# 1601339895/Image-Restoration

Measured on AMD Instinct MI355X. Metric: Mpixels/sec train (Restormer base 256x256, bs 32/GPU), higher is better.
Workload: dtype bf16; 1 GPU; Restormer base (dim 48, blocks [4,6,6,8], 26.13M params) train step: fwd + L1 + bwd + AdamW, 256x256 patches, bs 32/GPU, bf16 activations, fp32 params/grads/optimizer; per_gpu_batch=32, global_batch=32, patch=256, parallelism=dp1, hip_graph=False

## Files before the change

image_restoration_amd/_lib.py:

```python
from __future__ import annotations

import ctypes as C
import os
from typing import Optional

HERE = os.path.dirname(os.path.abspath(__file__))
LIB_PATH = os.environ.get("MI_RESTORE_LIB") or os.path.join(HERE, "libmi_restore.so")

MI_F32, MI_BF16 = 0, 1
c_i64 = C.c_int64
vp = C.c_void_p
fp = C.c_void_p


class PwDesc(C.Structure):
    _fields_ = [("x1", vp), ("x1_bs", c_i64), ("x1_gs", c_i64), ("k1", C.c_int),
                ("x2", vp), ("x2_bs", c_i64), ("x2_gs", c_i64), ("k2", C.c_int),
                ("w", fp), ("w_bs", c_i64), ("w_gs", c_i64), ("w_sm", c_i64), ("w_sk", c_i64),
                ("bias", fp), ("bias_gs", c_i64),
                ("r", vp), ("r_bs", c_i64), ("r_gs", c_i64),
                ("y", vp), ("y_bs", c_i64), ("y_gs", c_i64),
                ("m", C.c_int), ("n", c_i64), ("batch", C.c_int), ("groups", C.c_int), ("dtype", C.c_int),
                ("ln_w", fp), ("ln_b", fp), ("ln_mean", fp), ("ln_rstd", fp), ("ln_mode", C.c_int),
                ("f8", C.c_int), ("f8_sx", C.c_float), ("f8_sw", C.c_float),
# ... 189 lines not shown
    "mi_gdfn_fwd_f8_ok": (C.c_int, [C.POINTER(GdfnShape), C.c_int]),
    "mi_gdfn_fwd_f8": (C.c_int, [C.POINTER(GdfnShape), C.POINTER(GdfnParams), C.POINTER(LnHead), C.POINTER(F8Scales), vp, vp, vp,
                                 vp, vp]),
    "mi_box_down": (C.c_int, [vp, vp, C.c_int, C.c_int, C.c_int, C.c_int, C.c_int, C.c_int, vp]),
    "mi_fre_rect": (C.c_int, [fp, fp, fp, vp, C.c_int, C.c_int, C.c_int, C.c_int, C.c_int, C.c_int, vp]),
    "mi_fre_split_coef_bytes": (C.c_size_t, [C.c_int, C.c_int]),
    "mi_fre_split_workspace": (C.c_size_t, [C.c_int, C.c_int, C.c_int, C.c_int]),
    "mi_fre_split_max_hw": (C.c_int, []),
    "mi_fre_split_fwd": (C.c_int, [vp, vp, vp, vp, fp, C.c_int, C.c_int, C.c_int, C.c_int, C.c_int, vp]),
    "mi_fre_split_bwd": (C.c_int, [vp, vp, fp, vp, vp, vp, C.c_int, C.c_int, C.c_int, C.c_int, C.c_int, vp, vp]),
    "mi_chan_maxmean_fwd": (C.c_int, [vp, vp, vp, C.c_int, C.c_int, c_i64, C.c_int, vp]),
    "mi_chan_maxmean_bwd": (C.c_int, [vp, vp, vp, C.c_int, C.c_int, c_i64, C.c_int, vp]),
    "mi_plane_max_fwd": (C.c_int, [vp, fp, vp, C.c_int, c_i64, C.c_int, vp]),
    "mi_pool_pair_bwd": (C.c_int, [fp, fp, vp, vp, C.c_int, c_i64, C.c_int, vp]),
    "mi_chan_gate_fwd": (C.c_int, [fp, fp, fp, fp, fp, fp, C.c_int, C.c_int, C.c_int, vp]),
    "mi_chan_gate_bwd": (C.c_int, [fp, fp, fp, fp, fp, fp, fp, fp, fp, fp, fp, C.c_int, C.c_int, C.c_int, C.c_int, vp]),
    "mi_refine_mix_fwd": (C.c_int, [vp, vp, vp, fp, vp, C.c_int, C.c_int, c_i64, C.c_int, vp]),
    "mi_refine_mix_bwd": (C.c_int, [vp, vp, vp, fp, vp, vp, vp, vp, fp, C.c_int, C.c_int, c_i64, C.c_int, vp]),
    "mi_scale_add_fwd": (C.c_int, [vp, vp, fp, fp, vp, C.c_int, C.c_int, c_i64, C.c_int, vp]),
    "mi_scale_add_bwd": (C.c_int, [vp, vp, fp, fp, vp, vp, vp, fp, fp, C.c_int, C.c_int, c_i64, C.c_int, C.c_int, vp]),
    "mi_bwd_tail_ok": (C.c_int, [C.c_int, C.c_int, c_i64, C.c_int]),
    "mi_bwd_tail_workspace": (C.c_size_t, [C.c_int, C.c_int]),
    "mi_bwd_tail_plan": (C.c_int, [C.c_int, C.c_int, C.c_int, c_i64, C.c_int, C.POINTER(c_i64)]),
    "mi_bwd_tail": (C.c_int, [vp, C.c_int, vp, C.c_int, vp, fp, fp, fp, fp, fp, vp, fp, fp, fp, C.c_int, c_i64, C.c_int,
                              C.c_int, vp, vp]),
    "mi_mdta_bwd_ln_ok": (C.c_int, [C.POINTER(MdtaShape), C.c_int]),
    "mi_mdta_bwd_ln_workspace": (C.c_size_t, [C.POINTER(MdtaShape)]),
    "mi_mdta_bwd_ln": (C.c_int, [C.POINTER(MdtaShape), C.POINTER(MdtaParams), C.POINTER(LnTail), vp, vp, vp,
                                 C.POINTER(MdtaGrads), vp, vp, vp]),
    "mi_gdfn_bwd_ln_ok": (C.c_int, [C.POINTER(GdfnShape), C.c_int]),
    "mi_gdfn_bwd_ln_workspace": (C.c_size_t, [C.POINTER(GdfnShape)]),
    "mi_gdfn_bwd_ln": (C.c_int, [C.POINTER(GdfnShape), C.POINTER(GdfnParams), C.POINTER(LnTail), vp, vp, vp,
                                 C.POINTER(GdfnGrads), vp, vp, vp]),
    "mi_gdfn_fwd": (C.c_int, [C.POINTER(GdfnShape), C.POINTER(GdfnParams), vp, vp, vp, vp, vp, vp]),
    "mi_gdfn_bwd": (C.c_int, [C.POINTER(GdfnShape), C.POINTER(GdfnParams), vp, vp, vp, C.POINTER(GdfnGrads), vp, vp,
                              vp]),
    "mi_tksa_saved_bytes": (C.c_size_t, [C.POINTER(TksaShape)]),
    "mi_tksa_workspace": (C.c_size_t, [C.POINTER(TksaShape)]),
    "mi_tksa_fwd": (C.c_int, [C.POINTER(TksaShape), C.POINTER(MdtaParams), C.POINTER(TksaParams), vp, vp, vp, vp, vp, fp, vp]),
    "mi_tksa_bwd": (C.c_int, [C.POINTER(TksaShape), C.POINTER(MdtaParams), C.POINTER(TksaParams), vp, vp, vp, C.POINTER(MdtaGrads),
                              C.POINTER(TksaGrads), vp, vp, vp]),
    "mi_msfn_saved_bytes": (C.c_size_t, [C.POINTER(MsfnShape)]),
    "mi_msfn_workspace": (C.c_size_t, [C.POINTER(MsfnShape)]),
    "mi_msfn_fwd": (C.c_int, [C.POINTER(MsfnShape), C.POINTER(MsfnParams), vp, vp, vp, vp, vp, vp]),
    "mi_msfn_bwd": (C.c_int, [C.POINTER(MsfnShape), C.POINTER(MsfnParams), vp, vp, vp, C.POINTER(MsfnGrads), vp, vp, vp]),
    "mi_mefc_saved_bytes": (C.c_size_t, [C.POINTER(MefcShape)]),
# ... 91 lines not shown
```

image_restoration_amd/csrc/bwd_tail.hip:

```cpp
#include <limits.h>
#include <stdlib.h>

#include <type_traits>

#include <atomic>

#include "internal.h"
#include "fused_common.h"

namespace mi {
namespace {
using namespace fz;

#ifndef BT_PS_ELEMS
#define BT_PS_ELEMS 72
#endif
constexpr int BT_PS = BT_PS_ELEMS;

struct BtArgs {
  const bf16* dy;
  const bf16* x;
  const bf16* dres;
  const float* mean;
  const float* rstd;
// ... 14 lines not shown
  static constexpr int CT = C / 16;
  static constexpr int ROWS = 16 * MPW;
  static constexpr int KS = (ROWS + 31) / 32;
  static constexpr int PROWS = 32 * KS;
  static constexpr int NT = 64 * NW;
  static constexpr int XS = 68;

  static constexpr int LPP = NT / 64;
  static constexpr int CPL = C / LPP;
  static constexpr int ITEMS = C * 16 / NT;
  static constexpr int XP = C / 8;
  static constexpr int PPW = 2 * XP / NW;
  static constexpr int PATCH_E = PROWS * BT_PS;
  static constexpr int TILE_B = C * 128;
  static constexpr int OFF_XH = NW * PATCH_E * 2;
  static constexpr int OFF_DR = OFF_XH + 2 * TILE_B;
  static constexpr int OFF_ACC = OFF_DR + 2 * TILE_B;
  static constexpr int OFF_GAM = OFF_ACC + C * XS * 4;
  static constexpr int OFF_ST = OFF_GAM + C * 4;
  static constexpr int BYTES = OFF_ST + NW * 512;
  static_assert(C % 16 == 0 && (LPP == 4 || LPP == 8) && C % LPP == 0 && (C * 16) % NT == 0 && (2 * XP) % NW == 0,
                "unsupported shape");
  static_assert(C / 16 <= NW, "one wave per 16-channel output tile of the dxn product");
  static_assert(BYTES <= 160 * 1024, "LDS budget");
};


template <int C, int NW, int MPW>
__global__ __launch_bounds__(64 * NW, (BtCfg<C, NW, MPW>::BYTES <= 80 * 1024 ? 2 : 1)) void bt_kernel(BtArgs a) {
  using K = BtCfg<C, NW, MPW>;
  constexpr int CT = K::CT, KS = K::KS, PS = BT_PS, XS = K::XS, NT = K::NT, LPP = K::LPP, ITEMS = K::ITEMS;
  constexpr int XP = K::XP, PPW = K::PPW;
  extern __shared__ __attribute__((aligned(16))) unsigned char lds[];
  const int t = threadIdx.x, lane = t & 63, li = lane & 15, g = lane >> 4;
  const int wv = __builtin_amdgcn_readfirstlane(t >> 6);
  bf16* const patch = reinterpret_cast<bf16*>(lds) + wv * K::PATCH_E;
  float* const acc = reinterpret_cast<float*>(lds + K::OFF_ACC);
  float* const st = reinterpret_cast<float*>(lds + K::OFF_ST + wv * 512);
  const int m0 = wv * K::ROWS;
  const bool active = m0 < a.M;
  const u32x4 zero4 = {0u, 0u, 0u, 0u};
  const unsigned un = (unsigned)a.N;

  for (int i = lane; i < K::PATCH_E / 8; i += 64) reinterpret_cast<u32x4*>(patch)[i] = zero4;

  const bool dxn_wave = wv < CT;
  s16x8 wt[NW][KS];
#pragma unroll
  for (int o = 0; o < NW; ++o)
#pragma unroll
    for (int ks = 0; ks < KS; ++ks)
#pragma unroll
      for (int j = 0; j < 8; ++j) {
        const int ml = 32 * ks + (j < 4 ? 4 * g + j : 16 + 4 * g + j - 4), m = o * K::ROWS + ml;
        const bool ok = dxn_wave && ml < K::ROWS && m < a.M;
        const int cc = dxn_wave ? 16 * wv + li : 0;
        const float v = a.w[(ok ? m : 0) * C + cc] * a.gamma[cc];
        wt[o][ks][j] = ok ? bf_bits(v) : (short)0;
      }
  f32x4 G[MPW][CT];
  float S[MPW];
#pragma unroll
  for (int i = 0; i < MPW; ++i) {
    S[i] = 0.f;
#pragma unroll
    for (int ct = 0; ct < CT; ++ct) G[i][ct] = (f32x4){0.f, 0.f, 0.f, 0.f};
  }

  u32x4 R[MPW];
  const int rl = lane >> 2;
  auto issue_dy = [&](int tile, int h) {
    const int b = tile / a.tiles_per_image, p0 = (tile - b * a.tiles_per_image) * 64 + 32 * h;
    int ln = lane;
    asm volatile("" : "+v"(ln));
    const int rl = ln >> 2;
#pragma unroll
    for (int j = 0; j < MPW; ++j) {
      const int lim = a.M - 1 - (m0 + 16 * j);
      if (lim >= 0) {
        const bf16* base = a.dy + ((int64_t)b * a.M + m0 + 16 * j) * a.N + p0;
        const unsigned off = (unsigned)(rl < lim ? rl : lim) * un + 8u * (ln & 3);
        R[j] = *reinterpret_cast<const u32x4*>(base + off);
      }
    }
  };
  auto stage_dy = [&](int h) {
#pragma unroll
    for (int j = 0; j < MPW; ++j) {
      const int lim = a.M - 1 - (m0 + 16 * j);
      *reinterpret_cast<u32x4*>(&patch[(16 * j + rl) * PS + 32 * h + 8 * (lane & 3)]) = rl <= lim ? R[j] : zero4;
    }
// ... 30 lines not shown
    const bf16* b_lo = xh + li_ * 64 + ((k0 ^ f) << 3) + 4 * (g_ & 1);
    const bf16* b_hi = xh + li_ * 64 + (((k0 + 2) ^ f) << 3) + 4 * (g_ & 1);
#pragma unroll
    for (int i0 = 0; i0 < MPW; i0 += GRP) {
      s16x8 A[GRP];
#pragma unroll
      for (int i = 0; i < GRP; ++i) {
        const bf16* ar = ar0 + 16 * (i0 + i) * PS;
        A[i] = cat8(*reinterpret_cast<const s16x4*>(ar), *reinterpret_cast<const s16x4*>(ar + 16));
        float sm = 0.f;
#pragma unroll
        for (int j = 0; j < 8; ++j) sm += bf_s(A[i][j]);
        S[i0 + i] += sm;
      }
#pragma unroll
      for (int ct = 0; ct < CT; ++ct) {
        const s16x8 Bx = cat8(*reinterpret_cast<const s16x4*>(b_lo + ct * 16 * 64), *reinterpret_cast<const s16x4*>(b_hi + ct * 16 * 64));
#pragma unroll
        for (int i = 0; i < GRP; ++i) G[i0 + i][ct] = mfma32(A[i], Bx, G[i0 + i][ct]);
      }
    }
  };
  auto dxn_tile = [&]() {
    int ln = lane;
    asm volatile("" : "+v"(ln));
    const int li_ = ln & 15, g_ = ln >> 4, qq_ = li_ >> 2, pp_ = li_ & 3;
    f32x4 d[4];
#pragma unroll
    for (int nt = 0; nt < 4; ++nt) d[nt] = (f32x4){0.f, 0.f, 0.f, 0.f};
    const bf16* tr0 = reinterpret_cast<const bf16*>(lds) + (4 * g_ + qq_) * PS + 4 * pp_;
#pragma unroll
    for (int o = 0; o < NW; ++o) {
      if (o * K::ROWS < a.M) {
#pragma unroll
        for (int ks = 0; ks < KS; ++ks) {
          s16x4 lo[4], hi[4];
#pragma unroll
          for (int nt = 0; nt < 4; ++nt) {
            lo[nt] = tr_b16(tr0 + o * K::PATCH_E + (32 * ks) * PS + 16 * nt);
            hi[nt] = tr_b16(tr0 + o * K::PATCH_E + (32 * ks + 16) * PS + 16 * nt);
          }
          lds_wait(lo[0], hi[0], lo[1], hi[1], lo[2], hi[2], lo[3], hi[3]);
#pragma unroll
          for (int nt = 0; nt < 4; ++nt) d[nt] = mfma32(cat8(lo[nt], hi[nt]), wt[o][ks], d[nt]);
        }
      }
    }
    float* const ap0 = &acc[(16 * wv + li_) * XS + 4 * g_];
#pragma unroll
    for (int nt = 0; nt < 4; ++nt) *reinterpret_cast<f32x4*>(ap0 + 16 * nt) = d[nt];
  };

  auto ln_phase = [&](const bf16* xh, bf16* dr, f32x2 rstd_p) {
    if (a.dbg & 8) return;
    int tt = t;
    asm volatile("" : "+v"(tt));
    constexpr int L2 = 2 * LPP, CPL2 = C / L2;
    static_assert(C % L2 == 0 && (L2 == 8 || L2 == 16), "pixel-pair LayerNorm phase");
    const int px0 = 2 * (tt / L2), sub = tt % L2;
    int base[2];
    base[0] = sub * 64 + ((((px0 >> 3) ^ (sub >> 1)) & 7) << 3) + (px0 & 7);
    base[1] = sub * 64 + ((((px0 >> 3) ^ (sub >> 1) ^ (L2 == 8 ? 4 : 0)) & 7) << 3) + (px0 & 7);
    const float* const ap = &acc[sub * XS + px0];
    f32x2 gv[CPL2], xv[CPL2], s1 = {0.f, 0.f}, s2 = {0.f, 0.f};
#pragma unroll
    for (int j = 0; j < CPL2; ++j) {
      gv[j] = *reinterpret_cast<const f32x2*>(ap + L2 * j * XS);
      const unsigned xb = *reinterpret_cast<const unsigned*>(xh + base[j & 1] + L2 * j * 64);
      xv[j] = (f32x2){bf_lo(xb), bf_hi(xb)};
      s1 += gv[j];
      s2 += gv[j] * xv[j];
    }
    auto dpp = [](float v, auto ctrl) {
// ... 15 lines not shown
      s1[e] = u1 * (1.0f / C); s2[e] = u2 * (1.0f / C);
    }
#pragma unroll
    for (int j = 0; j < CPL2; ++j) {
      unsigned* const slot = reinterpret_cast<unsigned*>(dr + base[j & 1] + L2 * j * 64);
      const unsigned rb = *slot;
      const f32x2 o = rstd_p * (gv[j] - s1 - xv[j] * s2);
      *slot = pack_bf2(o[0] + bf_lo(rb), o[1] + bf_hi(rb));
    }
  };
  auto store_phase = [&](const bf16* dr, int b, int p0) {
    if (a.dbg & 16) return;
    int tt = t;
    asm volatile("" : "+v"(tt));
    const int c0 = tt >> 4, q = tt & 15;
    static_assert((NT / 32) % 8 == 0, "row step of the store loop must keep the swizzle term");
    const bf16* src = dr + c0 * 64 + ((((q >> 1) ^ (c0 >> 1)) & 7) << 3) + 4 * (q & 1);
    bf16* const ob = a.dx + (int64_t)b * C * a.N + p0 + (unsigned)c0 * un + 4u * q;
#pragma unroll
    for (int i = 0; i < ITEMS; ++i)
      MI_STREAM_ST(reinterpret_cast<u32x2*>(ob + (unsigned)(NT / 16 * i) * un), *reinterpret_cast<const u32x2*>(src + NT / 16 * i * 64));
  };

#ifdef BT_STAMP
  unsigned long long tk[12] = {0, 0, 0, 0, 0, 0, 0, 0, 0, 0, 0, 0}, t_prev = fm_clock();
#define BT_TICK(i) { const unsigned long long tn_ = fm_clock(); tk[i] += tn_ - t_prev; t_prev = tn_; }
#else
#define BT_TICK(i)
#endif
  int tile = blockIdx.x;
  if (tile < a.ntiles) {
    if (active) issue_dy(tile, 0);
    issue_x(tile, 0);
  }
  __syncthreads();
  int buf = 0, pb = 0, pp0 = 0;
  bool have_prev = false;
  f32x2 rstd_prev = {0.f, 0.f};
  for (; tile < a.ntiles; tile += gridDim.x, buf ^= 1) {
    const int b = tile / a.tiles_per_image, p0 = (tile - b * a.tiles_per_image) * 64;
    const int nxt = tile + gridDim.x;
    bf16* const xh = reinterpret_cast<bf16*>(lds + K::OFF_XH + buf * K::TILE_B);
    bf16* const dr = reinterpret_cast<bf16*>(lds + K::OFF_DR + buf * K::TILE_B);
    bf16* const xh_prev = reinterpret_cast<bf16*>(lds + K::OFF_XH + (buf ^ 1) * K::TILE_B);
    bf16* const dr_prev = reinterpret_cast<bf16*>(lds + K::OFF_DR + (buf ^ 1) * K::TILE_B);
    BT_TICK(0);
    asm volatile("s_waitcnt vmcnt(0)" ::: "memory");
    BT_TICK(1);
    if (active) stage_dy(0);
#pragma unroll
    for (int k = 0; k < PPW; ++k) {
      const int pid = wv + NW * k;
// ... 17 lines not shown
    BT_TICK(2);
    __syncthreads();
    BT_TICK(3);
    if (active) issue_dy(tile, 1);
    if (have_prev) ln_phase(xh_prev, dr_prev, rstd_prev);
    BT_TICK(4);
    __syncthreads();
    BT_TICK(5);
    if (have_prev) store_phase(dr_prev, pb, pp0);
    BT_TICK(6);
    if (active && !(a.dbg & 32)) {
      wgrad_half(0, xh);
      BT_TICK(7);
      stage_dy(1);
      wave_sync();
      BT_TICK(8);
      if (nxt < a.ntiles) issue_dy(nxt, 0);
      wgrad_half(1, xh);
    }
    BT_TICK(9);
    __syncthreads();
    BT_TICK(10);
    if (nxt < a.ntiles) issue_x(nxt, buf ^ 1);
    if (dxn_wave && !(a.dbg & 34)) dxn_tile();
    BT_TICK(11);
    __syncthreads();
    have_prev = true; pb = b; pp0 = p0; rstd_prev = rstd_p;
  }
  if (have_prev) {
    const int lb = buf ^ 1;
    bf16* const xh_l = reinterpret_cast<bf16*>(lds + K::OFF_XH + lb * K::TILE_B);
    bf16* const dr_l = reinterpret_cast<bf16*>(lds + K::OFF_DR + lb * K::TILE_B);
    ln_phase(xh_l, dr_l, rstd_prev);
    __syncthreads();
    store_phase(dr_l, pb, pp0);
  }
#ifdef BT_STAMP
  if (lane == 0) {
    float* const gp = a.gpart + (int64_t)blockIdx.x * a.M * (C + 1) + wv * 16;
#pragma unroll
    for (int i = 0; i < 12; ++i) gp[i] = (float)tk[i];
  }
  return;
#endif
  if (active) {
    float* const gp = a.gpart + (int64_t)blockIdx.x * a.M * (C + 1);
#pragma unroll
    for (int i = 0; i < MPW; ++i) {
#pragma unroll
      for (int ct = 0; ct < CT; ++ct)
#pragma unroll
        for (int r = 0; r < 4; ++r) {
          const int m = m0 + 16 * i + 4 * g + r;
          if (m < a.M) gp[(int64_t)m * (C + 1) + 16 * ct + li] = G[i][ct][r];
        }
      float sv = S[i];
      sv += __shfl_xor(sv, 16);
      sv += __shfl_xor(sv, 32);
      const int m = m0 + 16 * i + li;
      if (g == 0 && m < a.M) gp[(int64_t)m * (C + 1) + C] = sv;
    }
  }
}

// ... 33 lines not shown
  }
}

static bool bt_form(int M, int C, BtPlan* p) {
  int nw, mpw;
  const int mt = (M + 15) / 16;
  if (C == 96) { nw = 8; mpw = mt <= 24 ? 3 : 4; if (mt > 32) return false; }
  else if (C == 48) { nw = 4; mpw = mt <= 12 ? 3 : 4; if (mt > 16) return false; }
  else return false;
  p->C = C; p->NW = nw; p->MPW = mpw; p->rows = 16 * mpw; p->mpad = 16 * nw * mpw;
  p->lds = C == 96 ? (mpw == 3 ? BtCfg<96, 8, 3>::BYTES : BtCfg<96, 8, 4>::BYTES)
                   : (mpw == 3 ? BtCfg<48, 4, 3>::BYTES : BtCfg<48, 4, 4>::BYTES);
  p->grid = C == 96 ? 256 : 512;
  return true;
}
}

BtPlan bwd_tail_plan(int M, int C, int B, int64_t N, int dtype) {
  BtPlan p = {};
  if (!(dtype == MI_BF16 && B > 0 && N > 0 && N % 64 == 0 && M >= 16 && bt_form(M, C, &p))) return BtPlan{};
  p.covered = true;
  const char* e = MI_ENV(MI_BT_WIDE);
  p.pays = !(C == 96 && p.MPW == 4) || !(e && atoi(e) == 0);
  p.tiles_per_image = N / 64;
  p.tiles = (int64_t)B * p.tiles_per_image;
  p.launch = (int)(p.tiles < p.grid ? p.tiles : p.grid);
  p.passes = (int)((p.tiles + p.launch - 1) / p.launch);
  p.active = (M + p.rows - 1) / p.rows;
  const size_t mc = (size_t)M * (C + 1);
  p.ws_bytes = align_up((size_t)p.grid * mc * 4, 256) + align_up(mc * 4, 256) + align_up((size_t)REDUCE_GROUPS * mc * 4, 256);
  return p;
}

bool bwd_tail_ok(int M, int C, int64_t N, int dtype) { return bwd_tail_plan(M, C, 1, N, dtype).covered; }
bool bwd_tail_pays(int M, int C) { return bwd_tail_plan(M, C, 1, 64, MI_BF16).pays; }
size_t bwd_tail_workspace(int M, int C) { return bwd_tail_plan(M, C, 1, 64, MI_BF16).ws_bytes; }

template <int C, int NW, int MPW>
static int bt_launch(const BtArgs& a, int grid, hipStream_t st) {
  using K = BtCfg<C, NW, MPW>;
  static std::atomic<unsigned> attr_set{0};
  int dev = 0;
  MI_CHECK_HIP(hipGetDevice(&dev));
  const unsigned bit = 1u << (dev & 31);
  if (!(attr_set.load(std::memory_order_relaxed) & bit)) {
    MI_CHECK_HIP(hipFuncSetAttribute(reinterpret_cast<const void*>(&bt_kernel<C, NW, MPW>),
                                     hipFuncAttributeMaxDynamicSharedMemorySize, K::BYTES));
    attr_set.fetch_or(bit, std::memory_order_relaxed);
  }
  hipLaunchKernelGGL((bt_kernel<C, NW, MPW>), dim3(grid), dim3(64 * NW), K::BYTES, st, a);
  MI_LAUNCH_CHECK();
  return MI_OK;
}

int launch_bwd_tail(const void* dy, int M, const void* x, int C, const void* dres, const float* mean, const float* rstd,
                    const float* w, const float* gamma, const float* beta, void* dx, float* dw, float* dgamma, float* dbeta,
                    int B, int64_t N, int accumulate, void* ws, hipStream_t st) {
  const BtPlan p = bwd_tail_plan(M, C, B, N, MI_BF16);
  MI_CHECK_ARG(p.covered && p.tiles <= INT_MAX, "bwd_tail: unsupported shape M=%d C=%d B=%d N=%lld", M, C, B, (long long)N);
  MI_CHECK_ARG(dy && x && mean && rstd && w && gamma && dx && dw && dgamma && ws, "bwd_tail: null pointer");
  MI_CHECK_ARG(aligned16(dy) && aligned16(x) && aligned16(dx) && (!dres || aligned16(dres)) && aligned16(mean) && aligned16(rstd),
               "bwd_tail: operands must be 16-byte aligned");
  const size_t mc = (size_t)M * (C + 1);
  Carver cv(ws);
  float* gpart = cv.take<float>((size_t)p.grid * mc * 4);
  float* gsum = cv.take<float>(mc * 4);
  float* tmp = cv.take<float>((size_t)REDUCE_GROUPS * mc * 4);
  BtArgs a;
  a.dy = (const bf16*)dy; a.x = (const bf16*)x; a.dres = (const bf16*)dres; a.mean = mean; a.rstd = rstd; a.w = w;
  a.gamma = gamma; a.dx = (bf16*)dx; a.gpart = gpart; a.M = M; a.mpad = p.mpad; a.N = N;
  a.tiles_per_image = (int)p.tiles_per_image; a.ntiles = (int)p.tiles;
  { const char* e = MI_ENV(MI_BT_DEBUG); a.dbg = e ? atoi(e) : 0; }
  const int grid = p.launch;
  {
    const double px = (double)B * N;
    ProfScope ps(st, K_BWD_TAIL, ((double)M + 3.0 * C) * px * 2 + 8.0 * px, 4.0 * M * C * px);
    if (C == 96 && p.MPW == 4) MI_TRY((bt_launch<96, 8, 4>(a, grid, st)));
    else if (C == 96) MI_TRY((bt_launch<96, 8, 3>(a, grid, st)));
    else if (p.MPW == 4) MI_TRY((bt_launch<48, 4, 4>(a, grid, st)));
    else MI_TRY((bt_launch<48, 4, 3>(a, grid, st)));
  }
  (void)gsum;
  float* gb = accumulate ? deferred_take((size_t)M * 2 * C, st) : nullptr;
  if (!gb) gb = tmp;
  {
    ProfScope ps(st, K_BWD_TAIL_FIN, 4.0 * (grid + 2.0) * mc, (double)grid * mc);
    hipLaunchKernelGGL(bt_finish2_kernel, dim3(M), dim3(1024), 0, st, gpart, grid, w, gamma, beta, dw, gb, M, C, accumulate);
    MI_LAUNCH_CHECK();
  }
  if (dbeta) MI_TRY(launch_reduce_rows(gb, dgamma, M, 2 * C, 2 * C, accumulate, 1.0f, st, nullptr, dbeta, C));
  else MI_TRY(launch_reduce_rows(gb, dgamma, M, C, 2 * C, accumulate, 1.0f, st, nullptr, nullptr, 0));
  return MI_OK;
}

}

extern "C" int mi_bwd_tail_ok(int M, int C, int64_t N, int dtype) { return mi::bwd_tail_ok(M, C, N, dtype) ? 1 : 0; }
extern "C" size_t mi_bwd_tail_workspace(int M, int C) { return mi::bwd_tail_workspace(M, C); }
extern "C" int mi_bwd_tail_plan(int M, int C, int B, int64_t N, int dtype, int64_t* out) {
  MI_CHECK_ARG(out, "bwd_tail_plan: null pointer");
  MI_CHECK_ARG(dtype == MI_F32 || dtype == MI_BF16, "bwd_tail_plan: bad dtype %d", dtype);
  MI_CHECK_ARG(M > 0 && B > 0 && N > 0, "bwd_tail_plan: bad shape M=%d B=%d N=%lld", M, B, (long long)N);
  const mi::BtPlan p = mi::bwd_tail_plan(M, C, B, N, dtype);
  const int64_t v[12] = {p.covered, p.pays, p.NW, p.MPW, p.rows, p.mpad, p.launch, p.tiles, p.passes, p.active, (int64_t)p.lds,
                         (int64_t)p.ws_bytes};
  memcpy(out, v, sizeof(v));
  return MI_OK;
}
extern "C" int mi_bwd_tail(const void* dy, int M, const void* x, int C, const void* dres, const float* mean, const float* rstd,
                           const float* w, const float* gamma, const float* beta, void* dx, float* dw, float* dgamma,
                           float* dbeta, int B, int64_t N, int accumulate, int dtype, void* ws, void* stream) {
  MI_CHECK_ARG(dtype == MI_BF16, "bwd_tail: bf16 activations only");
  return mi::launch_bwd_tail(dy, M, x, C, dres, mean, rstd, w, gamma, beta, dx, dw, dgamma, dbeta, B, N, accumulate, ws,
                             (hipStream_t)stream);
}
```

image_restoration_amd/csrc/common.h:

```cpp
#pragma once
#include <hip/hip_runtime.h>
#include <stdint.h>
#include <stdio.h>
#include <string.h>
#include <type_traits>

#include "../../include/mi_restore.h"

namespace mi {

typedef __bf16 bf16;
typedef unsigned short u16;
typedef __attribute__((ext_vector_type(2))) float f32x2;
typedef __attribute__((ext_vector_type(4))) float f32x4;
typedef __attribute__((ext_vector_type(2))) unsigned int u32x2;
typedef __attribute__((ext_vector_type(4))) unsigned int u32x4;
typedef __attribute__((ext_vector_type(4))) short s16x4;
typedef __attribute__((ext_vector_type(8))) short s16x8;

template <bool F8> struct MfmaOp;
template <> struct MfmaOp<false> {
  using Frag = s16x8;
  static __device__ __forceinline__ void enter() {}
  static __device__ __forceinline__ Frag cvt(const s16x8 v, float) { return v; }
  static __device__ __forceinline__ f32x4 mma(Frag a, Frag b, f32x4 c) { return __builtin_amdgcn_mfma_f32_16x16x32_bf16(a, b, c, 0, 0, 0); }
};
template <> struct MfmaOp<true> {
  using Frag = long;
  typedef short s16x2_t __attribute__((ext_vector_type(2)));
  typedef __bf16 bf16x2_t __attribute__((ext_vector_type(2)));
  static __device__ __forceinline__ void enter() { __builtin_amdgcn_s_setreg((0 << 11) | (23 << 6) | 1, 1); }
  static __device__ __forceinline__ Frag cvt(const s16x8 v, float scale) {
    s16x2_t lo = {0, 0}, hi = {0, 0};
    lo = __builtin_amdgcn_cvt_scalef32_pk_fp8_bf16(lo, __builtin_bit_cast(bf16x2_t, (s16x2_t){v[0], v[1]}), scale, false);
    lo = __builtin_amdgcn_cvt_scalef32_pk_fp8_bf16(lo, __builtin_bit_cast(bf16x2_t, (s16x2_t){v[2], v[3]}), scale, true);
    hi = __builtin_amdgcn_cvt_scalef32_pk_fp8_bf16(hi, __builtin_bit_cast(bf16x2_t, (s16x2_t){v[4], v[5]}), scale, false);
    hi = __builtin_amdgcn_cvt_scalef32_pk_fp8_bf16(hi, __builtin_bit_cast(bf16x2_t, (s16x2_t){v[6], v[7]}), scale, true);
    return (long)(unsigned long)(unsigned)__builtin_bit_cast(int, lo) | ((long)__builtin_bit_cast(int, hi) << 32);
  }
  static __device__ __forceinline__ f32x4 mma(Frag a, Frag b, f32x4 c) { return __builtin_amdgcn_mfma_f32_16x16x32_fp8_fp8(a, b, c, 0, 0, 0); }
};

#define MI_ENV_LIST(X)                                                                                                       \
  X(MI_BT_WIDE) X(MI_BT_DEBUG) X(MI_DW_LDS) X(MI_FG_CFG) X(MI_FG_DEBUG) X(MI_FG_NOXCD) X(MI_GRAM_FOLD) X(MI_GRAM_WANT)      \
  X(MI_GRAM_RECT) X(MI_GRAM_LDS) X(MI_GRAM_STREAM_ALL) X(MI_LN_FORM) X(MI_CO_STREAM) X(MI_ATTN_DQK_SPLIT)    \
  X(MI_PW_DMA) X(MI_PW_TM_EVEN) X(MI_PW_WAVE) X(MI_PW_CHUNKED) X(MI_PW_XWIDE) X(MI_PW_WAVE_WIDE) X(MI_PW_DIRECT)             \
  X(MI_PW_WAVE_TPW) X(MI_PW_XCD) X(MI_PW_TPB) X(MI_PW_B16) X(MI_FM_DEBUG) X(MI_FM_CFG) X(MI_NO_FUSED_MDTA) X(MI_NO_PW_LDS) X(MI_PW_LDS)
enum EnvId {
#define MI_ENV_ENUM(n) E_##n,
  MI_ENV_LIST(MI_ENV_ENUM)
#undef MI_ENV_ENUM
  E_ENV_COUNT
};
const char* env_get(int id);
#define MI_ENV(n) ::mi::env_get(::mi::E_##n)

void set_error(const char* fmt, ...);
#define MI_CHECK_ARG(cond, ...)                \
  do {                                         \
    if (!(cond)) {                             \
      mi::set_error(__VA_ARGS__);              \
      return MI_ERR_ARG;                       \
    }                                          \
  } while (0)
#define MI_CHECK_HIP(expr)                                                          \
  do {                                                                              \
    hipError_t e_ = (expr);                                                         \
// ... 243 lines not shown
```

image_restoration_amd/csrc/internal.h:

```cpp
#pragma once
#include <initializer_list>

#include "common.h"

namespace mi {
struct PwK {
  const void* x1; int64_t x1_bs, x1_gs; int k1;
  const void* x2; int64_t x2_bs, x2_gs; int k2;
  const float* w; int64_t w_bs, w_gs, w_sm, w_sk;
  const float* bias; int64_t bias_gs;
  const void* r; int64_t r_bs, r_gs;
  void* y; int64_t y_bs, y_gs;
  int m; int64_t n; int groups; int vec_ok;
  void* y2; int64_t y2_bs, y2_gs; int y_split;
};
enum PwFamily { PW_CHUNKED = 0, PW_RESIDENT, PW_DMA, PW_XRES, PW_STREAM, PW_XWIDE, PW_LDS };
enum PwWeights { PW_W_PACK = 0, PW_W_B16, PW_W_F32 };
struct PwPlan {
  int family;
  int tm, m_tiles, k_chunks;
  bool f8, ln;
  bool vec_ok;
  int slices, per_batch, per_group, chunk_elems;
  int64_t slice_elems;
// ... 60 lines not shown
struct DwArgs {
  const void* in;
  const void* gy;
  const float* w;
  const float* bias;
  void* out;
  void* gate;
  int Cc, H, W, hidden, tiles_x;
};
bool dws_eligible(int H, int W, int ks);
int dws_partial_rows(int B, int H, int W, int64_t planes);
void dws_plan(int H, int W, int64_t planes, int* band, int* nb, int* lpr, int* uni);
int dws_fwd(const DwArgs& a, int B, bool gate, bool flip, int dtype, hipStream_t st);
int dws_bwd(const DwArgs& dya, const void* xin, float* part, int B, bool want_dx, int* rows_out, int dtype, hipStream_t st);
int dws_gate_bwd(const DwArgs& a, const void* xin, float* part, int B, bool want_dw, int* rows_out, int dtype,
                 hipStream_t st);
int dws_gate_bwd_recompute(const DwArgs& a, float* part, int B, bool want_dw, int* rows_out, int dtype, hipStream_t st);
struct BtPlan {
  bool covered, pays;
  int C, NW, MPW, rows, mpad;
  int grid, launch;
  int64_t tiles_per_image, tiles;
  int passes, active;
  size_t lds, ws_bytes;
};
BtPlan bwd_tail_plan(int M, int C, int B, int64_t N, int dtype);
bool bwd_tail_ok(int M, int C, int64_t N, int dtype);
bool bwd_tail_pays(int M, int C);
size_t bwd_tail_workspace(int M, int C);
int launch_bwd_tail(const void* dy, int M, const void* x, int C, const void* dres, const float* mean, const float* rstd,
                    const float* w, const float* gamma, const float* beta, void* dx, float* dw, float* dgamma, float* dbeta,
                    int B, int64_t N, int accumulate, void* ws, hipStream_t st);
#define MI_HIDDEN __attribute__((visibility("hidden")))
MI_HIDDEN int pw_lds_tm(int M);
MI_HIDDEN size_t pw_lds_lds_bytes(int tm);
MI_HIDDEN int pw_lds_launch(const mi_pw_desc* d, const PwPlan& pl, void* ws, hipStream_t st);
int fused_gdfn_fwd_save(const mi_gdfn_fused_shape* s, const void* pack, const void* y, void* out, float* mean, float* rstd,
                        void* h0, void* g, hipStream_t st);
enum FgEntry { FG_INFER = 0, FG_TRAIN, FG_F8 };
enum FgFamily { FG_TILE = 0, FG_FOURTH };
struct FgPlan {
  bool covered;
  int family;
  int C, th, tw, pc, nw; bool save, f8;
  int nch, ngr;
  int tiles_x, tiles_y, S;
// ... 68 lines not shown
```

image_restoration_amd/ops.py:

```python
from __future__ import annotations

import ctypes as C
import os
from typing import Optional, Sequence, Tuple

import torch

from . import _lib as L

Tensor = torch.Tensor


def _dtype_code(dtype: torch.dtype) -> int:
    if dtype == torch.float32:
        return L.MI_F32
    if dtype == torch.bfloat16:
        return L.MI_BF16
    raise TypeError(f"activations must be float32 or bfloat16, got {dtype}")


def _dt(t: Tensor) -> int:
    return _dtype_code(t.dtype)


# ... 766 lines not shown
    gg = _f32_struct(L.MefcGrads, grads[:5], "MEFC gradient", C.cast(ga, C.POINTER(L.MefcStepGrads)), int(accumulate))
    ws = _ws(lib.mi_mefc_workspace(C.byref(s)), x.device)
    L.check(lib.mi_mefc_bwd(C.byref(s), C.byref(pp), _p(x), _p(out), _p(dout), _p(dx), C.byref(gg), _p(saved), _p(ws), _stream()),
            "mefc_bwd")
    return dx


def bwd_tail_ok(M: int, Cc: int, N: int, dtype: torch.dtype) -> bool:
    return bool(L.lib().mi_bwd_tail_ok(M, Cc, N, _dtype_code(dtype)))


BWD_TAIL_PLAN_FIELDS = ("covered", "pays", "waves", "fragments", "rows_per_wave", "mpad", "workgroups", "tiles", "passes",
                        "active_waves", "lds", "workspace")


def bwd_tail_plan(M: int, Cc: int, B: int, N: int, dtype: torch.dtype) -> dict:
    out = (L.c_i64 * 12)()
    L.check(L.lib().mi_bwd_tail_plan(M, Cc, B, N, _dtype_code(dtype), out), "bwd_tail_plan")
    p = dict(zip(BWD_TAIL_PLAN_FIELDS, out))
    p["covered"], p["pays"] = bool(p["covered"]), bool(p["pays"])
    return p


def bwd_tail(dy: Tensor, x: Tensor, dres: Optional[Tensor], mean: Tensor, rstd: Tensor, w: Tensor, gamma: Tensor,
             beta: Tensor, dw: Tensor, dgamma: Tensor, dbeta: Tensor, accumulate: bool) -> Tensor:
    _gpu(dy, x, dres, mean, rstd, w, gamma, beta, dw, dgamma, dbeta)
    B, Cc, H, W = x.shape
    M = dy.shape[1]
    dx = torch.empty_like(x)
    lib = L.lib()
    ws = _ws(lib.mi_bwd_tail_workspace(M, Cc), x.device)
    L.check(lib.mi_bwd_tail(_p(dy), M, _p(x), Cc, _p(dres), _p(mean), _p(rstd), _p(w), _p(gamma), _p(beta), _p(dx), _p(dw),
                            _p(dgamma), _p(dbeta), B, H * W, int(accumulate), _dt(x), _p(ws), _stream()), "bwd_tail")
    return dx


def _gdfn_fused_shape(x: Tensor, hidden: int, with_bias: bool) -> L.GdfnFusedShape:
    B, Cc, H, W = x.shape
    return L.GdfnFusedShape(B, Cc, hidden, H, W, int(with_bias))


def gdfn_fused_ok(x: Tensor, hidden: int, ks: int = 3) -> bool:
    if x.dtype != torch.bfloat16 or ks != 3 or not x.is_cuda:
        return False
    s = _gdfn_fused_shape(x, hidden, True)
    return bool(L.lib().mi_gdfn_fused_ok(C.byref(s)))
# ... 717 lines not shown
```

include/mi_restore.h:

```cpp
#ifndef MI_RESTORE_H
#define MI_RESTORE_H

#include <stddef.h>
#include <stdint.h>

#ifdef __cplusplus
extern "C" {
#endif

#define MI_RESTORE_VERSION 100

typedef enum { MI_F32 = 0, MI_BF16 = 1 } mi_dtype;

enum {
  MI_OK = 0,
  MI_ERR_ARG = -1,
  MI_ERR_ALIGN = -2,
  MI_ERR_HIP = -3
};

int mi_version(void);
const char* mi_last_error(void);
int mi_env_reload(void);

// ... 202 lines not shown
                   void* out, void* saved, void* ws, void* stream);
typedef struct { float x1, w1, x2, w2; } mi_f8_scales;
int mi_mdta_fwd_f8_ok(const mi_mdta_shape* s, int with_ln);
int mi_mdta_fwd_f8(const mi_mdta_shape* s, const mi_mdta_params* p, const mi_ln_head* ln, const mi_f8_scales* f8, const void* x,
                   const void* residual, void* out, void* ws, void* stream);
int mi_gdfn_fwd_f8_ok(const mi_gdfn_shape* s, int with_ln);
int mi_gdfn_fwd_f8(const mi_gdfn_shape* s, const mi_gdfn_params* p, const mi_ln_head* ln, const mi_f8_scales* f8, const void* x,
                   const void* residual, void* out, void* ws, void* stream);
int mi_gdfn_fused_fwd_f8(const mi_gdfn_fused_shape* s, const void* pack, const mi_f8_scales* f8, const void* y, void* out,
                         void* stream);

int mi_mdta_fused_ok(const mi_mdta_shape* s);
int mi_mdta_fused_pays(const mi_mdta_shape* s);
size_t mi_mdta_fused_pack_bytes(const mi_mdta_shape* s);
int mi_mdta_fused_pack(const mi_mdta_shape* s, const float* ln_w, const float* ln_b, const mi_mdta_params* p, void* pack,
                       void* stream);
size_t mi_mdta_fused_workspace(const mi_mdta_shape* s);
int mi_mdta_fused_plan(const mi_mdta_shape* s, int64_t* out);
int mi_mdta_fused_fwd(const mi_mdta_shape* s, const mi_mdta_params* p, const void* pack, int ln_with_bias, const void* x,
                      const void* residual, void* out, float* mean, float* rstd, void* ws, void* stream);
int mi_bwd_tail_ok(int M, int C, int64_t N, int dtype);
size_t mi_bwd_tail_workspace(int M, int C);
int mi_bwd_tail_plan(int M, int C, int B, int64_t N, int dtype, int64_t* out);
int mi_bwd_tail(const void* dy, int M, const void* x, int C, const void* dres, const float* mean, const float* rstd,
                const float* w, const float* gamma, const float* beta, void* dx, float* dw, float* dgamma, float* dbeta,
                int B, int64_t N, int accumulate, int dtype, void* ws, void* stream);
int mi_mdta_bwd_ln_ok(const mi_mdta_shape* s, int qkv_bias);
size_t mi_mdta_bwd_ln_workspace(const mi_mdta_shape* s);
int mi_mdta_bwd_ln(const mi_mdta_shape* s, const mi_mdta_params* p, const mi_ln_tail* ln, const void* x, const void* dout,
                   void* dx, const mi_mdta_grads* gr, const void* saved, void* ws, void* stream);
int mi_gdfn_bwd_ln_ok(const mi_gdfn_shape* s, int in_bias);
size_t mi_gdfn_bwd_ln_workspace(const mi_gdfn_shape* s);
int mi_gdfn_bwd_ln(const mi_gdfn_shape* s, const mi_gdfn_params* p, const mi_ln_tail* ln, const void* x, const void* dout,
                   void* dx, const mi_gdfn_grads* gr, const void* saved, void* ws, void* stream);

int mi_box_down(const void* img, void* out, int B, int C, int Hi, int Wi, int factor, int dtype, void* stream);
int mi_fre_rect(const float* pooled, const float* w0, const float* w2, int* half, int B, int C, int R, int H, int W, int n,
                void* stream);
size_t mi_fre_split_coef_bytes(int B, int C);
size_t mi_fre_split_workspace(int B, int C, int H, int W);
int mi_fre_split_max_hw(void);
int mi_fre_split_fwd(const void* feat, const int* half, void* high, void* low, float* coef, int B, int C, int H, int W, int dtype,
                     void* stream);
int mi_fre_split_bwd(const void* feat, const int* half, const float* coef, const void* dhigh, const void* dlow, void* dfeat, int B,
                     int C, int H, int W, int dtype, void* ws, void* stream);
int mi_chan_maxmean_fwd(const void* x, void* out, int* idx, int B, int C, int64_t N, int dtype, void* stream);
// ... 120 lines not shown
```

Before: 15.82 Mpixels/s.

## Register-block the dxn product in bwd_tail across 2x4 waves for C=96

For C=96, the backward tail kernel's dxn matrix product is redistributed so every one of the 8 waves computes: waves split into 2 channel halves by 4 K-quarters. Each wave holds multiple 16-channel weight tiles in registers and reuses each transposed LDS load across them, then the partial sums are reduced into the shared accumulator over several sync rounds. This removes the idle waves of the old one-wave-per-channel-tile scheme and cuts redundant LDS reads. The cost is extra __syncthreads rounds, read-modify-write traffic on the accumulator, and higher register pressure. It is on by default for C=96 and can be turned off with an environment variable.

```diff
diff --git a/image_restoration_amd/_lib.py b/image_restoration_amd/_lib.py
--- a/image_restoration_amd/_lib.py
+++ b/image_restoration_amd/_lib.py
@@ -235,6 +235,7 @@
     "mi_bwd_tail_ok": (C.c_int, [C.c_int, C.c_int, c_i64, C.c_int]),
     "mi_bwd_tail_workspace": (C.c_size_t, [C.c_int, C.c_int]),
     "mi_bwd_tail_plan": (C.c_int, [C.c_int, C.c_int, C.c_int, c_i64, C.c_int, C.POINTER(c_i64)]),
+    "mi_bwd_tail_product": (C.c_int, [C.c_int, C.c_int, C.c_int, c_i64, C.c_int]),
     "mi_bwd_tail": (C.c_int, [vp, C.c_int, vp, C.c_int, vp, fp, fp, fp, fp, fp, vp, fp, fp, fp, C.c_int, c_i64, C.c_int,
                               C.c_int, vp, vp]),
     "mi_mdta_bwd_ln_ok": (C.c_int, [C.POINTER(MdtaShape), C.c_int]),
diff --git a/image_restoration_amd/csrc/bwd_tail.hip b/image_restoration_amd/csrc/bwd_tail.hip
--- a/image_restoration_amd/csrc/bwd_tail.hip
+++ b/image_restoration_amd/csrc/bwd_tail.hip
@@ -60,13 +60,17 @@
   static_assert(C % 16 == 0 && (LPP == 4 || LPP == 8) && C % LPP == 0 && (C * 16) % NT == 0 && (2 * XP) % NW == 0,
                 "unsupported shape");
   static_assert(C / 16 <= NW, "one wave per 16-channel output tile of the dxn product");
+  static constexpr int CTW = CT / 2;
+  static constexpr int KQ = NW / 2;
+  static constexpr int SPQ = NW * KS / KQ;
   static_assert(BYTES <= 160 * 1024, "LDS budget");
 };
 
 
-template <int C, int NW, int MPW>
+template <int C, int NW, int MPW, int RB>
 __global__ __launch_bounds__(64 * NW, (BtCfg<C, NW, MPW>::BYTES <= 80 * 1024 ? 2 : 1)) void bt_kernel(BtArgs a) {
   using K = BtCfg<C, NW, MPW>;
+  static_assert(!RB || (K::CT % 2 == 0 && NW % 2 == 0 && NW / 2 == 4 && (NW * K::KS) % 4 == 0), "register-blocked product: 2 x 4 waves");
   constexpr int CT = K::CT, KS = K::KS, PS = BT_PS, XS = K::XS, NT = K::NT, LPP = K::LPP, ITEMS = K::ITEMS;
   constexpr int XP = K::XP, PPW = K::PPW;
   extern __shared__ __attribute__((aligned(16))) unsigned char lds[];
@@ -82,20 +86,43 @@
 
   for (int i = lane; i < K::PATCH_E / 8; i += 64) reinterpret_cast<u32x4*>(patch)[i] = zero4;
 
-  const bool dxn_wave = wv < CT;
-  s16x8 wt[NW][KS];
-#pragma unroll
-  for (int o = 0; o < NW; ++o)
-#pragma unroll
-    for (int ks = 0; ks < KS; ++ks)
-#pragma unroll
-      for (int j = 0; j < 8; ++j) {
-        const int ml = 32 * ks + (j < 4 ? 4 * g + j : 16 + 4 * g + j - 4), m = o * K::ROWS + ml;
-        const bool ok = dxn_wave && ml < K::ROWS && m < a.M;
-        const int cc = dxn_wave ? 16 * wv + li : 0;
-        const float v = a.w[(ok ? m : 0) * C + cc] * a.gamma[cc];
-        wt[o][ks][j] = ok ? bf_bits(v) : (short)0;
-      }
+  const bool dxn_wave = RB || wv < CT;
+  s16x8 wt[RB ? 1 : NW][RB ? 1 : KS];
+  const int ch = wv & 1, kq = wv >> 1;
+  const int nreal = ((a.M + K::ROWS - 1) / K::ROWS) * KS, spq = (nreal + K::KQ - 1) / K::KQ;
+  s16x8 wt2[RB ? K::SPQ : 1][RB ? K::CTW : 1];
+  if constexpr (RB) {
+#pragma unroll
+    for (int s = 0; s < K::SPQ; ++s) {
+      const int f = kq * spq + s, o = f / KS, ks = f % KS;
+      const bool step = s < spq && f < nreal;
+#pragma unroll
+      for (int c3 = 0; c3 < K::CTW; ++c3) {
+        const int cc = 16 * (K::CTW * ch + c3) + li;
+        const float gm = a.gamma[cc];
+#pragma unroll
+        for (int j = 0; j < 8; ++j) {
+          const int ml = 32 * ks + (j < 4 ? 4 * g + j : 16 + 4 * g + j - 4), m = o * K::ROWS + ml;
+          const bool ok = step && ml < K::ROWS && m < a.M;
+          const float v = a.w[(ok ? m : 0) * C + cc] * gm;
+          wt2[s][c3][j] = ok ? bf_bits(v) : (short)0;
+        }
+      }
+    }
+  } else {
+#pragma unroll
+    for (int o = 0; o < NW; ++o)
+#pragma unroll
+      for (int ks = 0; ks < KS; ++ks)
+#pragma unroll
+        for (int j = 0; j < 8; ++j) {
+          const int ml = 32 * ks + (j < 4 ? 4 * g + j : 16 + 4 * g + j - 4), m = o * K::ROWS + ml;
+          const bool ok = dxn_wave && ml < K::ROWS && m < a.M;
+          const int cc = dxn_wave ? 16 * wv + li : 0;
+          const float v = a.w[(ok ? m : 0) * C + cc] * a.gamma[cc];
+          wt[o][ks][j] = ok ? bf_bits(v) : (short)0;
+        }
+  }
   f32x4 G[MPW][CT];
   float S[MPW];
 #pragma unroll
@@ -105,6 +132,14 @@
     for (int ct = 0; ct < CT; ++ct) G[i][ct] = (f32x4){0.f, 0.f, 0.f, 0.f};
   }
 
+#ifdef BT_STAMP
+  unsigned long long tk[14] = {0, 0, 0, 0, 0, 0, 0, 0, 0, 0, 0, 0, 0, 0}, t_prev = 0;
+#define BT_TICK_RESET() t_prev = fm_clock()
+#define BT_TICK(i) { const unsigned long long tn_ = fm_clock(); tk[i] += tn_ - t_prev; t_prev = tn_; }
+#else
+#define BT_TICK_RESET()
+#define BT_TICK(i)
+#endif
   u32x4 R[MPW];
   const int rl = lane >> 2;
   auto issue_dy = [&](int tile, int h) {
@@ -181,6 +216,7 @@
     }
   };
   auto dxn_tile = [&]() {
+    if constexpr (RB) return;
     int ln = lane;
     asm volatile("" : "+v"(ln));
     const int li_ = ln & 15, g_ = ln >> 4, qq_ = li_ >> 2, pp_ = li_ & 3;
@@ -201,13 +237,61 @@
           }
           lds_wait(lo[0], hi[0], lo[1], hi[1], lo[2], hi[2], lo[3], hi[3]);
 #pragma unroll
-          for (int nt = 0; nt < 4; ++nt) d[nt] = mfma32(cat8(lo[nt], hi[nt]), wt[o][ks], d[nt]);
+          for (int nt = 0; nt < 4; ++nt) d[nt] = mfma32(cat8(lo[nt], hi[nt]), wt[RB ? 0 : o][RB ? 0 : ks], d[nt]);
         }
       }
     }
     float* const ap0 = &acc[(16 * wv + li_) * XS + 4 * g_];
 #pragma unroll
     for (int nt = 0; nt < 4; ++nt) *reinterpret_cast<f32x4*>(ap0 + 16 * nt) = d[nt];
+  };
+
+  auto dxn_tile_rb = [&](bool run) {
+    if constexpr (RB) {
+      int ln = lane;
+      asm volatile("" : "+v"(ln));
+      const int li_ = ln & 15, g_ = ln >> 4, qq_ = li_ >> 2, pp_ = li_ & 3;
+      f32x4 d[4][K::CTW];
+#pragma unroll
+      for (int j = 0; j < 4; ++j)
+#pragma unroll
+        for (int c3 = 0; c3 < K::CTW; ++c3) d[j][c3] = (f32x4){0.f, 0.f, 0.f, 0.f};
+      const bf16* tr0 = reinterpret_cast<const bf16*>(lds) + (4 * g_ + qq_) * PS + 4 * pp_;
+      if (run) {
+#pragma unroll
+        for (int s = 0; s < K::SPQ; ++s) {
+          const int f = kq * spq + s;
+          if (s < spq && f < nreal) {
+            const bf16* tr = tr0 + (f / KS) * K::PATCH_E + 32 * (f % KS) * PS;
+            s16x4 lo[4], hi[4];
+#pragma unroll
+            for (int j = 0; j < 4; ++j) {
+              const int nt = (j + kq) & 3;
+              lo[j] = tr_b16(tr + 16 * nt);
+              hi[j] = tr_b16(tr + 16 * PS + 16 * nt);
+            }
+            lds_wait(lo[0], hi[0], lo[1], hi[1], lo[2], hi[2], lo[3], hi[3]);
+#pragma unroll
+            for (int j = 0; j < 4; ++j)
+#pragma unroll
+              for (int c3 = 0; c3 < K::CTW; ++c3) d[j][c3] = mfma32(cat8(lo[j], hi[j]), wt2[s][c3], d[j][c3]);
+          }
+        }
+      }
+      BT_TICK(12);
+      float* const ap0 = &acc[(16 * K::CTW * ch + li_) * XS + 4 * g_];
+#pragma unroll
+      for (int j = 0; j < 4; ++j) {
+        if (j) __syncthreads();
+        float* const ap = ap0 + 16 * ((j + kq) & 3);
+#pragma unroll
+        for (int c3 = 0; c3 < K::CTW; ++c3) {
+          f32x4* const p = reinterpret_cast<f32x4*>(ap + 16 * c3 * XS);
+          *p = j ? *p + d[j][c3] : d[j][c3];
+        }
+      }
+      BT_TICK(13);
+    }
   };
 
   auto ln_phase = [&](const bf16* xh, bf16* dr, f32x2 rstd_p) {
@@ -269,12 +353,7 @@
       MI_STREAM_ST(reinterpret_cast<u32x2*>(ob + (unsigned)(NT / 16 * i) * un), *reinterpret_cast<const u32x2*>(src + NT / 16 * i * 64));
   };
 
-#ifdef BT_STAMP
-  unsigned long long tk[12] = {0, 0, 0, 0, 0, 0, 0, 0, 0, 0, 0, 0}, t_prev = fm_clock();
-#define BT_TICK(i) { const unsigned long long tn_ = fm_clock(); tk[i] += tn_ - t_prev; t_prev = tn_; }
-#else
-#define BT_TICK(i)
-#endif
+  BT_TICK_RESET();
   int tile = blockIdx.x;
   if (tile < a.ntiles) {
     if (active) issue_dy(tile, 0);
@@ -338,7 +417,8 @@
     __syncthreads();
     BT_TICK(10);
     if (nxt < a.ntiles) issue_x(nxt, buf ^ 1);
-    if (dxn_wave && !(a.dbg & 34)) dxn_tile();
+    if constexpr (RB) dxn_tile_rb(!(a.dbg & 34));
+    else if (dxn_wave && !(a.dbg & 34)) dxn_tile();
     BT_TICK(11);
     __syncthreads();
     have_prev = true; pb = b; pp0 = p0; rstd_prev = rstd_p;
@@ -355,7 +435,7 @@
   if (lane == 0) {
     float* const gp = a.gpart + (int64_t)blockIdx.x * a.M * (C + 1) + wv * 16;
 #pragma unroll
-    for (int i = 0; i < 12; ++i) gp[i] = (float)tk[i];
+    for (int i = 0; i < 14; ++i) gp[i] = (float)tk[i];
   }
   return;
 #endif
@@ -435,6 +515,8 @@
   p.covered = true;
   const char* e = MI_ENV(MI_BT_WIDE);
   p.pays = !(C == 96 && p.MPW == 4) || !(e && atoi(e) == 0);
+  const char* rb = MI_ENV(MI_BT_REGBLOCK);
+  p.product = C == 96 && !(rb && atoi(rb) == 0) ? 2 : 1;
   p.tiles_per_image = N / 64;
   p.tiles = (int64_t)B * p.tiles_per_image;
   p.launch = (int)(p.tiles < p.grid ? p.tiles : p.grid);
@@ -449,7 +531,7 @@
 bool bwd_tail_pays(int M, int C) { return bwd_tail_plan(M, C, 1, 64, MI_BF16).pays; }
 size_t bwd_tail_workspace(int M, int C) { return bwd_tail_plan(M, C, 1, 64, MI_BF16).ws_bytes; }
 
-template <int C, int NW, int MPW>
+template <int C, int NW, int MPW, int RB>
 static int bt_launch(const BtArgs& a, int grid, hipStream_t st) {
   using K = BtCfg<C, NW, MPW>;
   static std::atomic<unsigned> attr_set{0};
@@ -457,11 +539,11 @@
   MI_CHECK_HIP(hipGetDevice(&dev));
   const unsigned bit = 1u << (dev & 31);
   if (!(attr_set.load(std::memory_order_relaxed) & bit)) {
-    MI_CHECK_HIP(hipFuncSetAttribute(reinterpret_cast<const void*>(&bt_kernel<C, NW, MPW>),
+    MI_CHECK_HIP(hipFuncSetAttribute(reinterpret_cast<const void*>(&bt_kernel<C, NW, MPW, RB>),
                                      hipFuncAttributeMaxDynamicSharedMemorySize, K::BYTES));
     attr_set.fetch_or(bit, std::memory_order_relaxed);
   }
-  hipLaunchKernelGGL((bt_kernel<C, NW, MPW>), dim3(grid), dim3(64 * NW), K::BYTES, st, a);
+  hipLaunchKernelGGL((bt_kernel<C, NW, MPW, RB>), dim3(grid), dim3(64 * NW), K::BYTES, st, a);
   MI_LAUNCH_CHECK();
   return MI_OK;
 }
@@ -488,10 +570,13 @@
   {
     const double px = (double)B * N;
     ProfScope ps(st, K_BWD_TAIL, ((double)M + 3.0 * C) * px * 2 + 8.0 * px, 4.0 * M * C * px);
-    if (C == 96 && p.MPW == 4) MI_TRY((bt_launch<96, 8, 4>(a, grid, st)));
-    else if (C == 96) MI_TRY((bt_launch<96, 8, 3>(a, grid, st)));
-    else if (p.MPW == 4) MI_TRY((bt_launch<48, 4, 4>(a, grid, st)));
-    else MI_TRY((bt_launch<48, 4, 3>(a, grid, st)));
+    if (C == 96 && p.product == 2) {
+      if (p.MPW == 4) MI_TRY((bt_launch<96, 8, 4, 1>(a, grid, st)));
+      else MI_TRY((bt_launch<96, 8, 3, 1>(a, grid, st)));
+    } else if (C == 96 && p.MPW == 4) MI_TRY((bt_launch<96, 8, 4, 0>(a, grid, st)));
+    else if (C == 96) MI_TRY((bt_launch<96, 8, 3, 0>(a, grid, st)));
+    else if (p.MPW == 4) MI_TRY((bt_launch<48, 4, 4, 0>(a, grid, st)));
+    else MI_TRY((bt_launch<48, 4, 3, 0>(a, grid, st)));
   }
   (void)gsum;
   float* gb = accumulate ? deferred_take((size_t)M * 2 * C, st) : nullptr;
@@ -520,6 +605,11 @@
   memcpy(out, v, sizeof(v));
   return MI_OK;
 }
+extern "C" int mi_bwd_tail_product(int M, int C, int B, int64_t N, int dtype) {
+  MI_CHECK_ARG(dtype == MI_F32 || dtype == MI_BF16, "bwd_tail_product: bad dtype %d", dtype);
+  MI_CHECK_ARG(M > 0 && B > 0 && N > 0, "bwd_tail_product: bad shape M=%d B=%d N=%lld", M, B, (long long)N);
+  return mi::bwd_tail_plan(M, C, B, N, dtype).product;
+}
 extern "C" int mi_bwd_tail(const void* dy, int M, const void* x, int C, const void* dres, const float* mean, const float* rstd,
                            const float* w, const float* gamma, const float* beta, void* dx, float* dw, float* dgamma,
                            float* dbeta, int B, int64_t N, int accumulate, int dtype, void* ws, void* stream) {
diff --git a/image_restoration_amd/csrc/common.h b/image_restoration_amd/csrc/common.h
--- a/image_restoration_amd/csrc/common.h
+++ b/image_restoration_amd/csrc/common.h
@@ -42,7 +42,7 @@
 };
 
 #define MI_ENV_LIST(X)                                                                                                       \
-  X(MI_BT_WIDE) X(MI_BT_DEBUG) X(MI_DW_LDS) X(MI_FG_CFG) X(MI_FG_DEBUG) X(MI_FG_NOXCD) X(MI_GRAM_FOLD) X(MI_GRAM_WANT)      \
+  X(MI_BT_WIDE) X(MI_BT_DEBUG) X(MI_BT_REGBLOCK) X(MI_DW_LDS) X(MI_FG_CFG) X(MI_FG_DEBUG) X(MI_FG_NOXCD) X(MI_GRAM_FOLD) X(MI_GRAM_WANT)      \
   X(MI_GRAM_RECT) X(MI_GRAM_LDS) X(MI_GRAM_STREAM_ALL) X(MI_LN_FORM) X(MI_CO_STREAM) X(MI_ATTN_DQK_SPLIT)    \
   X(MI_PW_DMA) X(MI_PW_TM_EVEN) X(MI_PW_WAVE) X(MI_PW_CHUNKED) X(MI_PW_XWIDE) X(MI_PW_WAVE_WIDE) X(MI_PW_DIRECT)             \
   X(MI_PW_WAVE_TPW) X(MI_PW_XCD) X(MI_PW_TPB) X(MI_PW_B16) X(MI_FM_DEBUG) X(MI_FM_CFG) X(MI_NO_FUSED_MDTA) X(MI_NO_PW_LDS) X(MI_PW_LDS)
diff --git a/image_restoration_amd/csrc/internal.h b/image_restoration_amd/csrc/internal.h
--- a/image_restoration_amd/csrc/internal.h
+++ b/image_restoration_amd/csrc/internal.h
@@ -106,6 +106,7 @@
   int grid, launch;
   int64_t tiles_per_image, tiles;
   int passes, active;
+  int product;
   size_t lds, ws_bytes;
 };
 BtPlan bwd_tail_plan(int M, int C, int B, int64_t N, int dtype);
diff --git a/image_restoration_amd/ops.py b/image_restoration_amd/ops.py
--- a/image_restoration_amd/ops.py
+++ b/image_restoration_amd/ops.py
@@ -812,6 +812,16 @@
     return p
 
 
+BWD_TAIL_PRODUCTS = {0: None, 1: "channel_tile", 2: "register_blocked"}
+
+
+def bwd_tail_product(M: int, Cc: int, B: int, N: int, dtype: torch.dtype) -> Optional[str]:
+    v = L.lib().mi_bwd_tail_product(M, Cc, B, N, _dtype_code(dtype))
+    if v < 0:
+        L.check(v, "bwd_tail_product")
+    return BWD_TAIL_PRODUCTS[v]
+
+
 def bwd_tail(dy: Tensor, x: Tensor, dres: Optional[Tensor], mean: Tensor, rstd: Tensor, w: Tensor, gamma: Tensor,
              beta: Tensor, dw: Tensor, dgamma: Tensor, dbeta: Tensor, accumulate: bool) -> Tensor:
     _gpu(dy, x, dres, mean, rstd, w, gamma, beta, dw, dgamma, dbeta)
diff --git a/include/mi_restore.h b/include/mi_restore.h
--- a/include/mi_restore.h
+++ b/include/mi_restore.h
@@ -248,6 +248,7 @@
 int mi_bwd_tail_ok(int M, int C, int64_t N, int dtype);
 size_t mi_bwd_tail_workspace(int M, int C);
 int mi_bwd_tail_plan(int M, int C, int B, int64_t N, int dtype, int64_t* out);
+int mi_bwd_tail_product(int M, int C, int B, int64_t N, int dtype);
 int mi_bwd_tail(const void* dy, int M, const void* x, int C, const void* dres, const float* mean, const float* rstd,
                 const float* w, const float* gamma, const float* beta, void* dx, float* dw, float* dgamma, float* dbeta,
                 int B, int64_t N, int accumulate, int dtype, void* ws, void* stream);
```

After: 15.87 Mpixels/s, median of 6. Within noise of the previous version (+0.3%).
